# 2bitoperations/rtldavis

Measured on AMD Instinct MI355X. Metric: complex MSamples/s demodulated (uint8 IQ -> packed bits -> preamble matches -> packets), higher is better.
Workload: dtype f32 (FIR: f16 x f16 -> f32 on the matrix pipe, exact integer accumulation); 1 GPU; 4096 streams x 33 blocks x 8192 samples uint8 IQ per GPU (BASELINE configs[3]/[4]: 64 unique synthetic streams tiled, 2.21 GB resident in HBM), 14 samples/symbol, 19.2 kbit/s; streams_per_gpu=4096, parallelism=streams/1

## Files before the change

rtldavis_amd/csrc/rd_demod_mfma.hip:

```cpp
#include <cstdio>
#include <cstdlib>
#include <cstring>

#include <hip/hip_ext.h>

#include "rd_internal.h"
#include "rd_math.h"
#include "rd_mfma.h"

#define RD_MF_WG 256
#define RD_MF_WAVES (RD_MF_WG / 64)
#ifndef RD_MF_MINWAVES
#define RD_MF_MINWAVES 4
#endif
#define RD_MF_GROUP_BYTES 1152
#define RD_MF_IMG_BYTES (16 + 4 * RD_MF_GROUP_BYTES)
#define RD_MF_IMG_PAD 4624
#define RD_MF_XB_BYTES (3 * 1024 + 32 + 32)
#define RD_MF_PEND 32
#ifndef RD_MF_STAGE_TILES
#define RD_MF_STAGE_TILES 4
#endif

typedef _Float16 rd_h8 __attribute__((ext_vector_type(8)));
typedef _Float16 rd_h16 __attribute__((ext_vector_type(16)));
typedef _Float16 rd_h2 __attribute__((ext_vector_type(2)));
typedef float rd_f16v __attribute__((ext_vector_type(16)));
typedef uint32_t rd_u4v __attribute__((ext_vector_type(4)));
typedef float rd_f4v __attribute__((ext_vector_type(4)));
typedef uint32_t rd_u2v __attribute__((ext_vector_type(2)));

static const rd_mf_taps h_mf_taps = rd_mf_make_taps();
__device__ const rd_mf_taps8 g_mf_taps8 = rd_mf_make_taps8();
static const rd_mf_taps8 h_mf_taps8 = rd_mf_make_taps8();
extern "C" void rd_debug_mfma_taps8(uint16_t *out) { memcpy(out, &h_mf_taps8, sizeof h_mf_taps8); }
#ifndef RD_MF_SPARSE
#define RD_MF_SPARSE 1
#endif
constexpr bool rd_mf_taps8s_ok() { bool ok = true; (void)rd_mf_make_taps8s(&ok); return ok; }
static_assert(rd_mf_taps8s_ok(), "a row of the tap matrix has more than two non-zero elements in a group of four");
constexpr rd_mf_taps8s rd_mf_taps8s_value() { bool ok = true; return rd_mf_make_taps8s(&ok); }
__device__ const rd_mf_taps8s g_mf_taps8s = rd_mf_taps8s_value();
static const rd_mf_taps8s h_mf_taps8s = rd_mf_taps8s_value();
extern "C" void rd_debug_mfma_taps8s(uint16_t *vals, uint32_t *idx) {
    memcpy(vals, h_mf_taps8s.v, sizeof h_mf_taps8s.v);
    memcpy(idx, h_mf_taps8s.idx, sizeof h_mf_taps8s.idx);
}

extern "C" void rd_debug_mfma_taps(uint16_t *out) { memcpy(out, &h_mf_taps, sizeof h_mf_taps); }

__device__ __forceinline__ rd_h8 rd_mf_frag(rd_u2v d) {
    rd_u4v v;
    v.x = d.x & 0x00FF00FFu;
    v.y = __builtin_amdgcn_perm(0u, d.x, 0x0c030c01u);
    v.z = d.y & 0x00FF00FFu;
    v.w = __builtin_amdgcn_perm(0u, d.y, 0x0c030c01u);
    return __builtin_bit_cast(rd_h8, v);
}

__device__ __forceinline__ float rd_mf_num(float ar, float ai, float cr, float ci, float &t1) {
    t1 = ai * ci;
    return __builtin_fmaf(-ar, cr, -t1);
}
__device__ __forceinline__ float rd_mf_guard(float nmin, float tmax) { return __builtin_fmaf(-4.76837158e-7f, tmax, nmin); }


template <int OFF>
__device__ __forceinline__ void rd_lds_write16(uint32_t addr, rd_f4v v) {
    asm volatile("ds_write_b128 %0, %1 offset:%2" : : "v"(addr), "v"(v), "i"(OFF) : "memory");
}
template <int OFF>
__device__ __forceinline__ rd_f4v rd_lds_read16(uint32_t addr) {
    rd_f4v r;
    asm volatile("ds_read_b128 %0, %1 offset:%2" : "=v"(r) : "v"(addr), "i"(OFF) : "memory");
    return r;
}
__device__ __forceinline__ void rd_lds_wait(rd_f4v &r) { asm volatile("s_waitcnt lgkmcnt(0)" : "+v"(r) : : "memory"); }
__device__ __forceinline__ void rd_lds_write4(uint32_t addr, uint32_t v) {
    asm volatile("ds_write_b32 %0, %1" : : "v"(addr), "v"(v) : "memory");
}
__device__ __forceinline__ rd_u4v rd_lds_read16u(uint32_t addr) {
    rd_u4v r;
    asm volatile("ds_read_b128 %0, %1\n\ts_waitcnt lgkmcnt(0)" : "=&v"(r) : "v"(addr) : "memory");
    return r;
}
__device__ __forceinline__ uint32_t rd_lds_read4(uint32_t addr) {
    uint32_t r;
    asm volatile("ds_read_b32 %0, %1\n\ts_waitcnt lgkmcnt(0)" : "=&v"(r) : "v"(addr) : "memory");
    return r;
}
__device__ __forceinline__ uint32_t rd_lds_addr(const void *p) {
    return (uint32_t)(uintptr_t)(const __attribute__((address_space(3))) void *)p;
}

__device__ __forceinline__ bool rd_mf_any(bool c) { return __ballot(c) != 0; }


struct rd_mf8_addr {
    uint32_t xw;
    uint32_t xw7;
    uint32_t rd1, rdE, rdO;
    uint32_t rd0;
};
struct rd_mf8_kept {
    float n2, n3;
    float g0r, g0i;
    float g1r, g1i, g2r, g2i;
    float nmin, tmax;
};

template <int B>
__device__ __forceinline__ constexpr int rd_mf8_woff() { return B == 0 ? 0 : (B & 1) ? 1024 : 2048; }

template <int B, int DBG>
__device__ __forceinline__ void rd_mf8_finish(const rd_mf8_kept &k, rd_f4v &p, uint32_t &W, uint32_t &fb, bool &slow) {
    rd_lds_wait(p);
    float t0, t1;
    const float n0 = rd_mf_num(p.x, p.y, p.z, p.w, t0);
    const float n1 = rd_mf_num(p.z, p.w, k.g0r, k.g0i, t1);
    if (DBG == 0 || DBG == 3) {
        const float nm = rd_mf_guard(rd_min3abs(k.nmin, n0, n1), rd_max3abs(k.tmax, t0, t1));
        if (rd_mf_any(!(nm > RD_MF_C0_MAX))) {
            slow = true;
            float F = rd_max3abs(0.0f, p.x, p.y);
            F = rd_max3abs(F, p.z, p.w);
            F = rd_max3abs(F, k.g0r, k.g0i);
            F = rd_max3abs(F, k.g1r, k.g1i);
            F = rd_max3abs(F, k.g2r, k.g2i);
            if (!(nm > rd_mf_c0(F))) fb |= 1u << (8 * (B & 3));
        }
    }
    uint32_t w = rd_shift_in_sign(W, n0);
    w = rd_shift_in_sign(w, n1);
    w = rd_shift_in_sign(w, k.n2);
    W = __builtin_amdgcn_alignbit(w, __builtin_bit_cast(uint32_t, k.n3), 27);
}

template <int B, int DBG>
__device__ __forceinline__ void rd_mf8_block(const rd_h8 (&A)[2], const rd_f16v &dcC, const int sidx, const int sidx2, const rd_u2v (&D)[9],
                                             rd_h8 &bfA, rd_h16 &bb, const rd_mf8_addr &ad, rd_mf8_kept &k0, rd_mf8_kept &kp, rd_f4v &p, uint32_t &Wlo,
                                             uint32_t &Whi, uint32_t &fblo, uint32_t &fbhi, bool &slow, float *dg, int dleft) {
    const rd_h8 bfB = rd_mf_frag(D[B + 1]);
    if (RD_MF_SPARSE && DBG != 8 && DBG != 9) {
        const rd_h16 wB = __builtin_shufflevector(bfB, bfB, 0, 1, 2, 3, 4, 5, 6, 7, 0, 1, 2, 3, 4, 5, 6, 7);
        if (B & 1) bb = __builtin_shufflevector(wB, bb, 0, 1, 2, 3, 4, 5, 6, 7, 24, 25, 26, 27, 28, 29, 30, 31);
        else bb = __builtin_shufflevector(bb, wB, 0, 1, 2, 3, 4, 5, 6, 7, 16, 17, 18, 19, 20, 21, 22, 23);
    }
    __builtin_amdgcn_sched_barrier(0);
    rd_f16v acc;
    if (DBG == 8 || DBG == 9) {
        rd_f16v c0 = dcC;
        if (DBG == 9) asm volatile("" : "+v"(c0));
        acc = __builtin_amdgcn_mfma_f32_32x32x16_f16(A[0], bfA, c0, 0, 0, 0);
        asm volatile("" : : "v"(bfB));
    } else if (RD_MF_SPARSE) {
        const uint32_t dbits = __builtin_bit_cast(uint32_t, -(float)RD_MF_DHI / 16777216.0f);
        uint64_t dh2 = ((uint64_t)dbits << 32) | dbits;
        asm volatile("" : "+s"(dh2));
        struct { uint64_t q[8]; } ci;
#pragma unroll
        for (int i = 0; i < 4; i++) asm volatile("v_mov_b64 %0, %1" : "=v"(ci.q[i]) : "s"(dh2));
#pragma unroll
        for (int i = 4; i < 8; i++) asm volatile("v_mov_b64 %0, 0" : "=v"(ci.q[i]));
        asm volatile("s_nop 1" ::: "memory");
        const rd_f16v c0 = __builtin_bit_cast(rd_f16v, ci);
        acc = (B & 1) ? __builtin_amdgcn_smfmac_f32_32x32x32_f16(A[1], bb, c0, sidx2, 0, 0)
                      : __builtin_amdgcn_smfmac_f32_32x32x32_f16(A[0], bb, c0, sidx, 0, 0);
    } else {
        acc = __builtin_amdgcn_mfma_f32_32x32x16_f16(A[0], bfA, dcC, 0, 0, 0);
        acc = __builtin_amdgcn_mfma_f32_32x32x16_f16(A[1], bfB, acc, 0, 0, 0);
    }
    if (B >= 2) rd_mf8_finish<B - 1, DBG>(kp, p, B - 1 <= 3 ? Wlo : Whi, B - 1 <= 3 ? fblo : fbhi, slow);
    __builtin_amdgcn_sched_barrier(0);
    float g[8];
#pragma unroll
    for (int i = 0; i < 8; i++) g[i] = __builtin_fmaf(acc[i], 2048.0f, acc[8 + i]);
    if (DBG == 3) {
#pragma unroll
        for (int r = 0; r < 4; r++)
            if (8 * B + r < dleft) { dg[2 * (8 * B + r)] = g[2 * r]; dg[2 * (8 * B + r) + 1] = g[2 * r + 1]; }
    }
    if (DBG != 10 && DBG != 11) {
        const rd_f4v x = {g[4], g[5], g[6], g[7]};
        if (B == 7) rd_lds_write16<0>(ad.xw7, x);
        else rd_lds_write16<rd_mf8_woff<B>()>(ad.xw, x);
    } else {
        asm volatile("" : : "v"(g[4]), "v"(g[5]), "v"(g[6]), "v"(g[7]));
    }
    if (B >= 1 && DBG != 10 && DBG != 11) p = rd_lds_read16<0>(B == 1 ? ad.rd1 : (B & 1) ? ad.rdO : ad.rdE);
    if (DBG == 11) asm volatile("" : "+v"(p));
    rd_mf8_kept &k = B == 0 ? k0 : kp;
    float t2, t3;
    k.n2 = rd_mf_num(g[0], g[1], g[2], g[3], t2);
    k.n3 = rd_mf_num(g[2], g[3], g[4], g[5], t3);
    k.nmin = rd_min3abs(3.0e38f, k.n2, k.n3);
    k.tmax = rd_max3abs(0.0f, t2, t3);
    k.g0r = g[0]; k.g0i = g[1];
    k.g1r = g[2]; k.g1i = g[3]; k.g2r = g[4]; k.g2i = g[5];
    bfA = bfB;
}

template <int DBG>
__device__ __forceinline__ void rd_mf8_tile(const rd_h8 (&A)[2], const rd_f16v &dcC, const int sidx, const int sidx2, const rd_u2v (&D)[9],
                                            const rd_mf8_addr &ad,
                                            uint32_t &word, uint32_t &fbw, bool &slow, float *dg, int dleft) {
    rd_h8 bfA = rd_mf_frag(D[0]);
    rd_h16 bb = __builtin_shufflevector(bfA, bfA, 0, 1, 2, 3, 4, 5, 6, 7, 8, 9, 10, 11, 12, 13, 14, 15);
    rd_mf8_kept k0, kp;
    rd_f4v p = {0.0f, 0.0f, 0.0f, 0.0f};
    uint32_t Wlo = 0, Whi = 0, fblo = 0, fbhi = 0;
    slow = false;
    rd_mf8_block<0, DBG>(A, dcC, sidx, sidx2, D, bfA, bb, ad, k0, kp, p, Wlo, Whi, fblo, fbhi, slow, dg, dleft);
    rd_mf8_block<1, DBG>(A, dcC, sidx, sidx2, D, bfA, bb, ad, k0, kp, p, Wlo, Whi, fblo, fbhi, slow, dg, dleft);
    rd_mf8_block<2, DBG>(A, dcC, sidx, sidx2, D, bfA, bb, ad, k0, kp, p, Wlo, Whi, fblo, fbhi, slow, dg, dleft);
    rd_mf8_block<3, DBG>(A, dcC, sidx, sidx2, D, bfA, bb, ad, k0, kp, p, Wlo, Whi, fblo, fbhi, slow, dg, dleft);
    rd_mf8_block<4, DBG>(A, dcC, sidx, sidx2, D, bfA, bb, ad, k0, kp, p, Wlo, Whi, fblo, fbhi, slow, dg, dleft);
    rd_mf8_block<5, DBG>(A, dcC, sidx, sidx2, D, bfA, bb, ad, k0, kp, p, Wlo, Whi, fblo, fbhi, slow, dg, dleft);
    rd_mf8_block<6, DBG>(A, dcC, sidx, sidx2, D, bfA, bb, ad, k0, kp, p, Wlo, Whi, fblo, fbhi, slow, dg, dleft);
    rd_mf8_block<7, DBG>(A, dcC, sidx, sidx2, D, bfA, bb, ad, k0, kp, p, Wlo, Whi, fblo, fbhi, slow, dg, dleft);
    rd_f4v p0 = rd_lds_read16<0>(ad.rd0);
    rd_mf8_finish<7, DBG>(kp, p, Whi, fbhi, slow);
    {
        rd_lds_wait(p0);
        float t0, t1;
        const float n0 = rd_mf_num(p0.x, p0.y, p0.z, p0.w, t0);
        const float n1 = rd_mf_num(p0.z, p0.w, k0.g0r, k0.g0i, t1);
        if (DBG == 0 || DBG == 3) {
            const float nm = rd_mf_guard(rd_min3abs(k0.nmin, n0, n1), rd_max3abs(k0.tmax, t0, t1));
            if (rd_mf_any(!(nm > RD_MF_C0_MAX))) {
                slow = true;
                float F = rd_max3abs(0.0f, p0.x, p0.y);
                F = rd_max3abs(F, p0.z, p0.w);
                F = rd_max3abs(F, k0.g0r, k0.g0i);
                F = rd_max3abs(F, k0.g1r, k0.g1i);
                F = rd_max3abs(F, k0.g2r, k0.g2i);
                if (!(nm > rd_mf_c0(F))) fblo |= 1u;
            }
        }
        uint32_t b0 = rd_shift_in_sign(0u, n0);
        b0 = rd_shift_in_sign(b0, n1);
        b0 = rd_shift_in_sign(b0, k0.n2);
        b0 = __builtin_amdgcn_alignbit(b0, __builtin_bit_cast(uint32_t, k0.n3), 27);
        Wlo = (b0 << 24) | Wlo;
    }
    const uint32_t Vlo = __builtin_bitreverse32(Wlo & 0xF0F0F0F0u), Vhi = __builtin_bitreverse32(Whi & 0xF0F0F0F0u);
    const auto r = __builtin_amdgcn_permlane32_swap(Vlo, Vhi, false, false);
    word = (r[1] << 4) | r[0];
    fbw = 0;
    if (slow && rd_mf_any((fblo | fbhi) != 0)) {
        const auto f = __builtin_amdgcn_permlane32_swap(fblo, fbhi, false, false);
        fbw = f[0] | f[1];
    }
}

#ifndef RD_MF_LOAD_AUX
#define RD_MF_LOAD_AUX 2
#endif

__device__ __forceinline__ void rd_mf_issue(const rd_layout &lay, uint32_t s, uint32_t ti, uint8_t *img, int lane,
                                            bool halo_dma = true) {
    const uint8_t *src = lay.iq + (size_t)s * lay.stream_stride + (size_t)ti * RD_TILE_BYTES;
    const int perm = 8 * (lane & 7) + (lane >> 3);
    const __attribute__((address_space(1))) void *g0 = (const __attribute__((address_space(1))) void *)(src + perm * 16);
    __builtin_amdgcn_global_load_lds(g0, (__attribute__((address_space(3))) void *)(img + 16), 16, 0, RD_MF_LOAD_AUX);
    __builtin_amdgcn_global_load_lds(g0, (__attribute__((address_space(3))) void *)(img + 16 + 128), 16, 1024, RD_MF_LOAD_AUX);
    __builtin_amdgcn_global_load_lds(g0, (__attribute__((address_space(3))) void *)(img + 16 + 256), 16, 2048, RD_MF_LOAD_AUX);
    __builtin_amdgcn_global_load_lds(g0, (__attribute__((address_space(3))) void *)(img + 16 + 384), 16, 3072, RD_MF_LOAD_AUX);
    const bool has_halo = (ti > 0) || lay.hist_mode;
    if (lane == 0 && halo_dma)
        __builtin_amdgcn_global_load_lds((const __attribute__((address_space(1))) void *)(src + (has_halo ? -16 : 0)),
                                         (__attribute__((address_space(3))) void *)(img), 16, 0, 0);
}

__device__ __forceinline__ int rd_lane_now() {
    return (int)__builtin_amdgcn_mbcnt_hi(~0u, __builtin_amdgcn_mbcnt_lo(~0u, 0u));
}

__device__ __forceinline__ void rd_mf_flush(const uint32_t *pend, uint32_t count, uint32_t *fix_list, uint32_t fix_cap,
                                            uint32_t *counters, uint32_t bits_stride, uint32_t *bucket_cnt) {
    const int lane = rd_lane_now();
    asm volatile("s_waitcnt lgkmcnt(0)" ::: "memory");
    if (bucket_cnt) {
        for (uint32_t i = lane; i < count; i += 64) {
            const uint32_t e = pend[i];
            const uint32_t grp = ((e >> 4) / bits_stride) >> RD_FT_GSH;
            const uint32_t slot = atomicAdd(&bucket_cnt[grp], 1u);
            if (slot < fix_cap) fix_list[(size_t)grp * fix_cap + slot] = e;
        }
        return;
    }
    uint32_t base = 0;
    if (lane == 0) base = atomicAdd(&counters[RD_CNT_FIX], count);
    base = __builtin_amdgcn_readfirstlane(base);
    for (uint32_t i = lane; i < count; i += 64)
        if (base + i < fix_cap) fix_list[base + i] = pend[i];
}


__device__ __forceinline__ void rd_mf_store_staged(uint32_t stage_addr, uint32_t nst, uint32_t *base, uint32_t stflags) {
    const int lane = rd_lane_now();
    if (nst == RD_MF_STAGE_TILES) {
#pragma unroll
        for (int j = 0; j < RD_MF_STAGE_TILES / 4; j++) {
            const rd_u4v v = rd_lds_read16u(stage_addr + 16 * (lane + 64 * j));
            if (!(stflags & 1)) __builtin_nontemporal_store(v, (rd_u4v *)(base + 4 * (lane + 64 * j)));
            else *(rd_u4v *)(base + 4 * (lane + 64 * j)) = v;
        }
    } else {
        for (uint32_t q = 0; q < nst; q++) base[64 * q + lane] = rd_lds_read4(stage_addr + 256 * q + 4 * lane);
    }
}

struct rd_mf_pos {
    uint32_t tile, s, ti, inchunk;
};
struct rd_mf_nextchunk {
    uint32_t tile, s, ti;
};
__device__ __forceinline__ rd_mf_nextchunk rd_mf_chunk_at(uint64_t chunk_id, uint32_t chunk, uint32_t tps, uint32_t total) {
    rd_mf_nextchunk c;
    const uint32_t n_chunks = (total + chunk - 1) / chunk;
    const bool have = chunk_id < n_chunks;
    const uint32_t nt = have ? (uint32_t)chunk_id * chunk : 0u;
    c.tile = have ? nt : 0xFFFFFFFFu;
    c.s = 0; c.ti = 0;
    if (have) {
        c.s = __builtin_amdgcn_readfirstlane(c.tile / tps);
        c.ti = c.tile - c.s * tps;
    }
    return c;
}
__device__ __forceinline__ rd_mf_pos rd_mf_next(rd_mf_pos p, uint32_t chunk, uint32_t tps, const rd_mf_nextchunk &nc) {
    rd_mf_pos q;
    if (p.inchunk + 1 < chunk) {
        q.tile = p.tile + 1; q.inchunk = p.inchunk + 1;
        q.s = p.s; q.ti = p.ti + 1;
        if (q.ti >= tps) { q.ti = 0; q.s++; }
    } else {
        q.tile = nc.tile; q.inchunk = 0;
        q.s = nc.s; q.ti = nc.ti;
    }
    return q;
}

__device__ __forceinline__ void rd_mf_read_window(uint32_t a_prv, uint32_t a_own, rd_u2v (&D)[9]) {
    asm volatile("ds_read_b64 %0, %9\n\t"
                 "ds_read_b64 %1, %10\n\t"
                 "ds_read_b64 %2, %10 offset:128\n\t"
                 "ds_read_b64 %3, %10 offset:256\n\t"
                 "ds_read_b64 %4, %10 offset:384\n\t"
                 "ds_read_b64 %5, %10 offset:512\n\t"
                 "ds_read_b64 %6, %10 offset:640\n\t"
                 "ds_read_b64 %7, %10 offset:768\n\t"
                 "ds_read_b64 %8, %10 offset:896\n\t"
                 "s_waitcnt lgkmcnt(0)"
                 : "=&v"(D[0]), "=&v"(D[1]), "=&v"(D[2]), "=&v"(D[3]), "=&v"(D[4]), "=&v"(D[5]), "=&v"(D[6]),
                   "=&v"(D[7]), "=&v"(D[8])
                 : "v"(a_prv), "v"(a_own)
                 : "memory");
}

__device__ __forceinline__ uint64_t rd_stamp() {
    uint64_t t;
    __builtin_amdgcn_sched_barrier(0);
    asm volatile("s_memtime %0\n\ts_waitcnt lgkmcnt(0)" : "=s"(t) : : "memory");
    __builtin_amdgcn_sched_barrier(0);
    return t;
}
__device__ __forceinline__ uint64_t rd_stamp_real() {
    uint64_t t;
    __builtin_amdgcn_sched_barrier(0);
    asm volatile("s_memrealtime %0\n\ts_waitcnt lgkmcnt(0)" : "=s"(t) : : "memory");
    __builtin_amdgcn_sched_barrier(0);
    return t;
}


#define RD_STAMP_WORDS 12
#define RD_STF_BUCKETS 8192u
template <int DBG, bool STAMP>
__global__ __launch_bounds__(RD_MF_WG, RD_MF_MINWAVES) void k_demod_mfma(rd_layout lay, uint32_t tiles_per_stream, uint32_t total_tiles,
                                                         uint32_t chunk, uint32_t *fix_list, uint32_t fix_cap,
                                                         uint32_t *counters, float *dbg_g, uint32_t stflags) {
    __shared__ __attribute__((aligned(16))) uint8_t s_img[RD_MF_WAVES][RD_MF_IMG_PAD];
    __shared__ __attribute__((aligned(32))) uint8_t s_xb[RD_MF_WAVES][RD_MF_XB_BYTES];
    __shared__ uint32_t s_pend[RD_MF_WAVES][RD_MF_PEND];
    __shared__ __attribute__((aligned(16))) uint32_t s_stage[RD_MF_WAVES][RD_MF_STAGE_TILES][64];
    constexpr bool LOADS = DBG != 1;
    const int lane = threadIdx.x & 63;
    const int wave = __builtin_amdgcn_readfirstlane(threadIdx.x >> 6);
    uint8_t *img0 = s_img[wave];
    uint8_t *xb = s_xb[wave];
    uint32_t *mypend = s_pend[wave];
    uint32_t npend = 0;
    constexpr bool CAN_BUCKET = DBG == 0 && !STAMP;
    uint32_t *bucket_cnt = (CAN_BUCKET && (stflags & RD_STF_BUCKETS)) ? (uint32_t *)dbg_g : nullptr;

    const int n = lane & 31, h = lane >> 5;
    rd_h8 A8[2];
    rd_f16v dcC;
    int sidx = 0, sidx2 = 0;
    if (RD_MF_SPARSE && DBG != 8 && DBG != 9) {
        A8[0] = *(const rd_h8 *)g_mf_taps8s.v[lane];
        A8[1] = *(const rd_h8 *)g_mf_taps8s.v[lane ^ 32];
        sidx = (int)g_mf_taps8s.idx[lane];
        sidx2 = (int)g_mf_taps8s.idx[lane ^ 32];
    } else {
        A8[0] = *(const rd_h8 *)g_mf_taps8.v[0][lane];
        A8[1] = *(const rd_h8 *)g_mf_taps8.v[1][lane];
    }
    const float dchi = -(float)RD_MF_DHI / 16777216.0f;
#pragma unroll
    for (int i = 0; i < 16; i++) dcC[i] = i < 8 ? dchi : 0.0f;
    if (RD_MF_SPARSE && DBG != 8 && DBG != 9) asm volatile("" : "+v"(A8[0]), "+v"(A8[1]), "+v"(sidx), "+v"(sidx2));
    else asm volatile("" : "+v"(A8[0]), "+v"(A8[1]), "+v"(dcC));
    const uint32_t img_addr = rd_lds_addr(img0);
    const uint32_t own = 16 + RD_MF_GROUP_BYTES * (n >> 3) + 16 * (n & 7) + 8 * h;
    const uint32_t prv = n == 0 ? 8 * h
                       : (n & 7) ? own + 16 * 55
                                 : 16 + RD_MF_GROUP_BYTES * ((n >> 3) - 1) + 16 * 63 + 8 * h;
    const uint32_t xb_addr = rd_lds_addr(xb), pend_addr = rd_lds_addr(mypend);
    const uint32_t stage_addr = rd_lds_addr(s_stage[wave]);
    const uint32_t rtoggle = lane == 0 ? 16u : 0u, wtoggle = lane == 63 ? 16u : 0u;
    rd_mf8_addr ad8;
    ad8.xw = xb_addr + 16 * lane;
    ad8.xw7 = xb_addr + (lane == 63 ? 3072 : 1024 + 16 * lane);
    ad8.rd1 = xb_addr + (h ? 1024 + 16 * (lane - 32) : 16 * (lane + 32));
    ad8.rdE = xb_addr + (h ? 2048 + 16 * (lane - 32) : 1024 + 16 * (lane + 32));
    ad8.rdO = xb_addr + (h ? 1024 + 16 * (lane - 32) : 2048 + 16 * (lane + 32));
    ad8.rd0 = xb_addr + (h ? 16 * (lane - 32) : lane ? 1024 + 16 * (lane + 31) : 3072 + 16);
    if (lane < 8) ((uint32_t *)(xb + 3072))[lane] = 0;

    const uint32_t nwaves = gridDim.x * RD_MF_WAVES;
    const uint32_t wave_id = blockIdx.x * RD_MF_WAVES + wave;
    const bool dynamic = !(stflags & 4096) && chunk >= 4;
    uint32_t cur_chunk = wave_id;
    rd_mf_nextchunk nextc = {0xFFFFFFFFu, 0, 0};
    if (!dynamic) nextc = rd_mf_chunk_at((uint64_t)cur_chunk + nwaves, chunk, tiles_per_stream, total_tiles);
    uint32_t grab = 0;
    bool grab_pending = false;
    const uint32_t my_queue = wave_id % RD_NQUEUE;
    uint32_t *queue = &counters[RD_CNT_QUEUE0 + RD_QUEUE_STRIDE * my_queue];
    rd_mf_pos cur;
    cur.tile = wave_id * chunk;
    cur.s = cur.tile / tiles_per_stream;
    cur.ti = cur.tile % tiles_per_stream;
    cur.inchunk = 0;
    rd_mf_pos nx1 = rd_mf_next(cur, chunk, tiles_per_stream, nextc);

    uint32_t nst = 0;
    uint32_t *st_base = nullptr;
    bool st_flush = false;
    uint64_t sm_wait = 0, sm_gap = 0, sm_comp = 0, sm_wait_st = 0, sm_t0 = 0, sm_r0 = 0, sm_mark = 0, sm_wmax = 0;
    uint32_t sm_iters = 0, sm_iters_st = 0;
    bool sm_stored = false;
    if (STAMP) { sm_t0 = rd_stamp(); sm_r0 = rd_stamp_real(); }
    if (LOADS && cur.tile < total_tiles) rd_mf_issue(lay, cur.s, cur.ti, img0, lane);
    if (STAMP) sm_mark = rd_stamp();
    while (cur.tile < total_tiles) {
        const uint32_t tile = cur.tile, s = cur.s, ti = cur.ti, inchunk = cur.inchunk;
        uint64_t sm_a = 0;
        if (STAMP) { sm_a = rd_stamp(); sm_comp += sm_a - sm_mark; }
        asm volatile("s_waitcnt vmcnt(0)" : "+v"(grab) : : "memory");
        uint64_t sm_b = 0;
        if (STAMP) {
            sm_b = rd_stamp();
            const uint64_t w = sm_b - sm_a;
            sm_wait += w;
            if (w > sm_wmax) sm_wmax = w;
            if (sm_stored) { sm_wait_st += w; sm_iters_st++; }
            sm_iters++;
            sm_stored = false;
        }
        if (dynamic) {
            if (grab_pending) {
                nextc = rd_mf_chunk_at((uint64_t)nwaves + my_queue + (uint64_t)RD_NQUEUE * __builtin_amdgcn_readfirstlane(grab),
                                       chunk, tiles_per_stream, total_tiles);
                grab_pending = false;
            }
            if (inchunk == 0) {
                const uint32_t one = 1, zoff = 0;
                uint64_t saved_exec;
                asm volatile("s_mov_b64 %1, exec\n\ts_mov_b64 exec, 1\n\tglobal_atomic_add %0, %2, %3, %4 sc0\n\ts_mov_b64 exec, %1"
                             : "+v"(grab), "=&s"(saved_exec) : "v"(zoff), "v"(one), "s"(queue) : "memory");
                grab_pending = true;
            }
        } else if (inchunk == 0 && tile != wave_id * chunk) {
            cur_chunk += nwaves;
            nextc = rd_mf_chunk_at((uint64_t)cur_chunk + nwaves, chunk, tiles_per_stream, total_tiles);
        }
        if (!(stflags & 4)) __builtin_amdgcn_s_setprio(3);
        rd_u2v D[9];
        rd_mf_read_window(img_addr + prv, img_addr + own, D);
        if (nst == RD_MF_STAGE_TILES || (nst && st_flush)) {
            rd_mf_store_staged(stage_addr, nst, st_base, stflags);
            nst = 0;
            if (STAMP) sm_stored = true;
        }
        const rd_mf_pos nx2 = rd_mf_next(nx1, chunk, tiles_per_stream, nextc);
        bool halo_dma = true;
        {
            const bool follows = nx1.tile < total_tiles && nx1.s == s && nx1.ti == ti + 1;
            if (follows) {
                halo_dma = false;
                if (n == 31) asm volatile("ds_write_b64 %0, %1" : : "v"(img_addr + 8 * h), "v"(D[8]) : "memory");
            }
        }
        if (LOADS && nx1.tile < total_tiles) rd_mf_issue(lay, nx1.s, nx1.ti, img0, lane, halo_dma);
        if (!(stflags & 4)) __builtin_amdgcn_s_setprio(0);
        if (STAMP) { sm_mark = rd_stamp(); sm_gap += sm_mark - sm_b; }

        uint32_t word = 0;
        bool slow_taken = false;
        uint32_t fbw8 = 0;
        if (DBG == 2 || DBG == 6) {
#pragma unroll
            for (int j = 0; j < 9; j++) word ^= D[j].x ^ D[j].y;
        } else {
            float *dg = DBG == 3 ? dbg_g + ((size_t)tile * RD_TILE_SAMPLES + 64 * n + 4 * h + 1) * 2 : nullptr;
            const int dleft = RD_TILE_SAMPLES - (64 * n + 4 * h + 1);
            rd_mf8_tile<DBG>(A8, dcC, sidx, sidx2, D, ad8, word, fbw8, slow_taken, dg, dleft);
            ad8.rd0 ^= rtoggle;
            ad8.xw7 ^= wtoggle;
        }
        uint32_t gmask = 0;
        const bool carry = inchunk > 0 && ti > 0;
        const uint32_t run = ti * 64 + 2 * n + h;
        const uint32_t t0 = run * RD_RUN;
        const bool any_flag = slow_taken && rd_mf_any(fbw8 != 0);
        if (any_flag) gmask = ((fbw8 * 0x00204081u) >> 21) & 0xFu;
        if (!carry && lane == 0) {
            if (ti == 0 && !lay.hist_mode) gmask = 0xFu;
            else gmask |= 1u;
        }
        const bool ragged = (ti + 1 == tiles_per_stream) && (lay.n_samples % RD_TILE_SAMPLES) != 0;
        if (DBG == 6) {
            if (word == 0x12345678u) lay.bits[0] = word;
        } else if (!ragged) {
            if (nst == 0) {
                st_base = &lay.bits[(size_t)s * lay.bits_stride + ti * 64];
                if (stflags & 2) st_base = &lay.bits[(((size_t)s * lay.bits_stride + ti * 64) & 0x3FFFFu) & ~255u];
            }
            rd_lds_write4(stage_addr + 256 * nst + 4 * (2 * n + h), word);
            nst++;
            const bool next_ragged = (nx1.ti + 1 == tiles_per_stream) && (lay.n_samples % RD_TILE_SAMPLES) != 0;
            st_flush = !(nx1.tile < total_tiles && nx1.s == s && nx1.ti == ti + 1 && !next_ragged);
        } else if (t0 < lay.n_samples) {
            const uint32_t left = lay.n_samples - t0;
            if (left < RD_RUN) {
                word &= (1u << left) - 1u;
                gmask &= (1u << ((left + RD_GROUP - 1) / RD_GROUP)) - 1u;
            }
            lay.bits[(size_t)s * lay.bits_stride + run] = word;
        } else {
            gmask = 0;
        }
        if (DBG == 1 || DBG == 2 || DBG == 6) gmask = 0;
        const uint64_t fm = (any_flag || !carry) ? __ballot(gmask != 0) : 0;
        if (fm) {
            const uint32_t nf = (uint32_t)__popcll(fm);
            if (npend + nf > RD_MF_PEND) {
                rd_mf_flush(mypend, npend, fix_list, fix_cap, counters, (uint32_t)lay.bits_stride, bucket_cnt);
                npend = 0;
            }
            if (gmask)
                rd_lds_write4(pend_addr + 4 * (npend + __builtin_amdgcn_mbcnt_hi((uint32_t)(fm >> 32),
                                                                                  __builtin_amdgcn_mbcnt_lo((uint32_t)fm, 0))),
                              ((uint32_t)((size_t)s * lay.bits_stride + run) << 4) | gmask);
            npend += nf;
        }
        cur = nx1;
        nx1 = nx2;
    }
    if (nst) rd_mf_store_staged(stage_addr, nst, st_base, stflags);
    if (npend) rd_mf_flush(mypend, npend, fix_list, fix_cap, counters, (uint32_t)lay.bits_stride, bucket_cnt);
    if (STAMP && dbg_g) {
        const uint64_t t1 = rd_stamp(), r1 = rd_stamp_real();
        sm_comp += t1 - sm_mark;
        if (lane == 0) {
            uint64_t *o = (uint64_t *)dbg_g + (size_t)wave_id * RD_STAMP_WORDS;
            o[0] = sm_wait; o[1] = sm_gap; o[2] = sm_comp; o[3] = sm_wait_st;
            o[4] = sm_iters; o[5] = sm_iters_st; o[6] = t1 - sm_t0; o[7] = r1 - sm_r0;
            o[8] = sm_wmax; o[9] = sm_r0; o[10] = r1;
            uint32_t xcc;
            asm volatile("s_getreg_b32 %0, hwreg(HW_REG_XCC_ID)" : "=s"(xcc));
            o[11] = xcc;
        }
    }
}

static int rd_mf_env(const char *name, int dflt) {
    const char *e = getenv(name);
    return e ? atoi(e) : dflt;
}

struct rd_mf_params {
    int dbg = 0, stamp = 0, chunk_env = 0, per_cu_env = 0, n_cu = 256;
    uint32_t stflags = 0;
    rd_mf_params() {
        chunk_env = rd_mf_env("RD_K1_CHUNK", 0);
        per_cu_env = rd_mf_env("RD_K1_WGS_PER_CU", 0);
#ifdef RD_DIAG
        dbg = rd_mf_env("RD_K1_DEBUG", 0);
        stamp = rd_mf_env("RD_K1_STAMPS", 0) ? 1 : 0;
        stflags = (uint32_t)rd_mf_env("RD_K1_STFLAGS", 0) & (1u | 2u | 4u | 4096u);
#endif
        int dev = 0;
        hipDeviceProp_t prop;
        if (hipGetDevice(&dev) == hipSuccess && hipGetDeviceProperties(&prop, dev) == hipSuccess && prop.multiProcessorCount > 0)
            n_cu = prop.multiProcessorCount;
    }
};
static const rd_mf_params &rd_mf_get_params() {
    static const rd_mf_params p;
    return p;
}

#ifdef RD_DIAG
static uint64_t *g_stamp_buf = nullptr;
static uint32_t g_stamp_waves = 0;
extern "C" int rd_diag_read_stamps(uint64_t *out, uint32_t cap_waves, uint32_t *n_waves) {
    if (!g_stamp_buf || !n_waves) return RD_ERR_STATE;
    if (hipDeviceSynchronize() != hipSuccess) return RD_ERR_DEVICE;
    *n_waves = g_stamp_waves;
    const uint32_t n = g_stamp_waves < cap_waves ? g_stamp_waves : cap_waves;
    if (n && hipMemcpy(out, g_stamp_buf, (size_t)n * RD_STAMP_WORDS * 8, hipMemcpyDeviceToHost) != hipSuccess) return RD_ERR_DEVICE;
    return RD_OK;
}
extern "C" int rd_diag_variant(int *dbg, int *stamp, uint32_t *stflags) {
    const rd_mf_params &P = rd_mf_get_params();
    if (dbg) *dbg = P.dbg;
    if (stamp) *stamp = P.stamp;
    if (stflags) *stflags = P.stflags;
    return RD_OK;
}
#endif

struct rd_mf_launch_args {
    rd_layout lay;
    uint32_t tps, total;
    uint64_t total64;
// ... 145 lines not shown
```

rtldavis_amd/csrc/rd_kernels.hip:

```cpp
#include <algorithm>
#include <cstdlib>

#include <hip/hip_ext.h>

#include "rd_internal.h"
#include "rd_math.h"
#include "rd_mfma.h"
#include "rd_parse.h"

uint32_t rd_launch_demod(const rd_layout &lay, uint32_t *fix_list, uint32_t fix_cap, uint32_t *counters, hipStream_t st,
                         hipEvent_t ev_start, hipEvent_t ev_stop, uint32_t flags, uint32_t *chunk_out, uint32_t *bucket_cnt) {
    if (!bucket_cnt) flags &= ~RD_DEMOD_FIX_BUCKETS;
    const bool bucketed = rd_launch_demod_mfma(lay, fix_list, fix_cap, counters, st, ev_start, ev_stop, nullptr, flags, chunk_out, bucket_cnt);
    return bucketed ? RD_DEMOD_FIX_BUCKETS : 0u;
}

__global__ __launch_bounds__(256) void k_fixup(rd_layout lay, uint32_t runs_per_stream, const uint32_t *fix_list,
                                               uint32_t fix_cap, const uint32_t *counters, int all,
                                               uint32_t *zero_next, uint32_t zero_words) {
    if (zero_next && blockIdx.x == 0)
        for (uint32_t i = threadIdx.x; i < zero_words; i += blockDim.x) zero_next[i] = 0;
    uint64_t count;
    if (all) {
        count = (uint64_t)lay.n_streams * runs_per_stream;
// ... 791 lines not shown
}

#define RD_FT_WG 256
#ifndef RD_FT_DEPTH
#define RD_FT_DEPTH 5
#endif
struct rd_ft_args {
    rd_layout lay;
    rd_devcfg cfg;
    int n_calls;
    int p_hi;
    int skip_fix;
    const uint32_t *fixb;
    const uint32_t *fixcnt;
    uint32_t fix_bcap;
    uint32_t bcap;
    uint32_t bucket_limit;
    uint32_t *gstate;
    uint32_t seq;
    rd_packet *recs;
    uint32_t rec_cap;
    uint32_t *counters;
    uint32_t *zero_next;
    uint32_t zero_words;
    uint64_t *stamps;
    int abl;
};
#ifdef RD_DIAG
#define RD_FT_STAMP(k) do { if (a.stamps && (tid & 63) == 0) { uint64_t t_; asm volatile("s_memrealtime %0\n\ts_waitcnt lgkmcnt(0)" : "=s"(t_) : : "memory"); \
                                                               a.stamps[(size_t)grp * 8 + (k)] = t_; } } while (0)
#else
#define RD_FT_STAMP(k) do { } while (0)
#endif

template <int S_, int T>
__device__ __forceinline__ uint32_t rd_tap(const uint32_t *r, int o) {
    constexpr int wj = (T * S_) >> 5, sh = (T * S_) & 31;
    return sh ? __builtin_amdgcn_alignbit(r[o + wj + 1], r[o + wj], sh) : r[o + wj];
}
constexpr int rd_tt3(bool pa, bool pb, bool pc) { return (pa ? 0xF0 : 0x0F) & (pb ? 0xCC : 0x33) & (pc ? 0xAA : 0x55); }
template <int S_, int P_, uint64_t PRE_, int T>
__device__ __forceinline__ uint32_t rd_match_from(uint32_t m, const uint32_t *r, int o) {
    if constexpr (T >= P_) {
        return m;
    } else if constexpr (T + 1 == P_) {
        const uint32_t v = rd_tap<S_, T>(r, o);
        return __builtin_amdgcn_bitop3_b32(m, v, v, rd_tt3(true, (PRE_ >> T) & 1, (PRE_ >> T) & 1));
    } else {
        const uint32_t n = __builtin_amdgcn_bitop3_b32(m, rd_tap<S_, T>(r, o), rd_tap<S_, T + 1>(r, o),
                                                       rd_tt3(true, (PRE_ >> T) & 1, (PRE_ >> (T + 1)) & 1));
        return rd_match_from<S_, P_, PRE_, T + 2>(n, r, o);
    }
}
template <int S_, int P_, uint64_t PRE_>
__device__ __forceinline__ uint32_t rd_match_word(const uint32_t *r, int o) {
    static_assert(P_ >= 3, "three taps in the first instruction");
    const uint32_t m = __builtin_amdgcn_bitop3_b32(rd_tap<S_, 0>(r, o), rd_tap<S_, 1>(r, o), rd_tap<S_, 2>(r, o),
                                                   rd_tt3(PRE_ & 1, (PRE_ >> 1) & 1, (PRE_ >> 2) & 1));
    return rd_match_from<S_, P_, PRE_, 3>(m, r, o);
}

__device__ __forceinline__ void rd_barrier_lds() { asm volatile("s_waitcnt lgkmcnt(0)\n\ts_barrier" ::: "memory"); }

template <int S_, int P_, uint64_t PRE_, int K_>
__global__ __launch_bounds__(RD_FT_WG, 4) void k_tail(rd_ft_args a) {
    constexpr int G = RD_FT_STREAMS;
    static_assert(PRE_ & 1, "positions below 0 are skipped because the preamble starts with a one");
    static_assert(RD_FT_WG == 64 * G, "one wave per stream in the classify strips");
    extern __shared__ __attribute__((aligned(16))) uint32_t s_dyn[];
    uint32_t *s_t = s_dyn;
    int32_t *s_pos = (int32_t *)(s_dyn + (size_t)G * a.bcap * 8);
    uint32_t *s_ord = s_dyn + (size_t)G * a.bcap * 9;
    __shared__ uint32_t s_cnt[G], s_kept[G];
    __shared__ uint32_t s_ready;
    const int tid = threadIdx.x, lane = tid & 63, wave = __builtin_amdgcn_readfirstlane(tid >> 6);
    const int grp = blockIdx.x, n_groups = gridDim.x;
    const int stream0 = grp * G;
    const int n_here = a.lay.n_streams - stream0 < G ? a.lay.n_streams - stream0 : G;
    const int nwords = (int)((a.lay.n_samples + 31) / 32);
    if (grp == 0 && a.zero_next)
        for (uint32_t i = tid; i < a.zero_words; i += RD_FT_WG) a.zero_next[i] = 0;
    if (tid < G) { s_cnt[tid] = 0; s_kept[tid] = 0; }
    if (tid == 0) s_ready = 0;
    const int prio_q = (int)(((unsigned)grp * 4u) / (unsigned)n_groups);
    if (wave == 0) RD_FT_STAMP(0);

    uint32_t n_fix_raw = 0;
    if (!a.skip_fix) {
        const uint32_t *bk = a.fixb + (size_t)grp * a.fix_bcap;
        const uint32_t e_first = (uint32_t)tid < a.fix_bcap ? bk[tid] : 0u;
        n_fix_raw = a.fixcnt[grp];
        const uint32_t n_fix = n_fix_raw < a.fix_bcap ? n_fix_raw : a.fix_bcap;
        uint32_t *s_items = s_t;
        __shared__ uint32_t s_nitems;
        static_assert(RD_GROUPS == 4, "an entry lists up to four groups");
        for (uint32_t i0 = 0; i0 < n_fix; i0 += RD_FT_WG) {
            if (tid == 0) s_nitems = 0;
            __syncthreads();
            const uint32_t i = i0 + (uint32_t)tid;
            const uint32_t e = i < n_fix ? (i0 == 0 ? e_first : bk[i]) : 0u;
            const uint32_t k = (uint32_t)__popc(e & 0xFu);
            if (k) {
                uint32_t at = atomicAdd(&s_nitems, k);
                for (int g = 0; g < RD_GROUPS; g++)
                    if ((e >> g) & 1) s_items[at++] = ((uint32_t)tid << 2) | (uint32_t)g;
                s_items[4 * RD_FT_WG + tid] = e;
            }
            __syncthreads();
            const uint32_t n_items = s_nitems;
            for (uint32_t it = (uint32_t)tid; it < n_items; it += RD_FT_WG) {
                const uint32_t item = s_items[it];
                const uint32_t ee = s_items[4 * RD_FT_WG + (item >> 2)];
                const int g = (int)(item & 3u);
                const uint32_t widx = ee >> 4;
                const uint32_t s = widx / (uint32_t)a.lay.bits_stride;
                const uint32_t run = widx - s * (uint32_t)a.lay.bits_stride;
                const uint8_t *base = a.lay.iq + (size_t)s * a.lay.stream_stride;
                const long t0 = (long)run * RD_RUN + g * RD_GROUP;
                const long left = (long)a.lay.n_samples - t0;
                if (left <= 0) continue;
                const int count = left < RD_GROUP ? (int)left : RD_GROUP;
                const uint8_t *p = base + 2 * (t0 - 10);
                uint32_t dw[10];
                const long x = a.lay.valid_from - (t0 - 10), z = (long)a.lay.n_samples + 8 - (t0 - 10);
                const int d_lo = x <= 0 ? 0 : x >= 20 ? 10 : (int)(x / 2);
                const int d_hi = z <= 0 ? 0 : z >= 20 ? 10 : (int)((z + 1) / 2);
#pragma unroll
                for (int d = 0; d < 10; d++) dw[d] = (d >= d_lo && d < d_hi) ? *(const uint32_t *)(p + 4 * d) : 0u;
                ((uint8_t *)a.lay.bits)[(size_t)widx * 4 + g] = (uint8_t)rd_exact_group_dw(dw, t0, count, a.lay.valid_from);
            }
            if (i0 + RD_FT_WG < n_fix) __syncthreads();
        }
    }
    __syncthreads();
    if (wave == 0) RD_FT_STAMP(1);

    {
        constexpr int NW = ((RD_SEARCH_OUT + ((P_ - 1) * S_ + 31) / 32 + 1 + 3) / 4) * 4;
        const int gps = a.p_hi / (32 * RD_SEARCH_OUT) + 1;
        const int wgps = (gps + 63) / 64;
        const int units = n_here * wgps;
        auto fetch = [&](int g, int rem, uint32_t (&r)[NW]) {
            const int gi = rem * 64 + lane;
            const uint32_t *w = a.lay.bits + (size_t)(stream0 + g) * a.lay.bits_stride;
            int w0 = RD_SEARCH_OUT * gi;
            w0 = w0 + NW <= nwords ? w0 : nwords - NW;
#pragma unroll
            for (int j = 0; j < NW / 4; j++) {
                const uint4 v4 = *(const uint4 *)(w + w0 + 4 * j);
                r[4 * j] = v4.x; r[4 * j + 1] = v4.y; r[4 * j + 2] = v4.z; r[4 * j + 3] = v4.w;
            }
        };
        auto test = [&](int g, int rem, const uint32_t (&r)[NW]) {
            const int gi = rem * 64 + lane;
            uint32_t m[RD_SEARCH_OUT] = {};
            const int p0 = 32 * RD_SEARCH_OUT * gi;
            if (gi < gps) {
#pragma unroll
                for (int o = 0; o < RD_SEARCH_OUT; o++) m[o] = rd_match_word<S_, P_, PRE_>(r, o);
                if (p0 + 32 * RD_SEARCH_OUT - 1 > a.p_hi) {
#pragma unroll
                    for (int o = 0; o < RD_SEARCH_OUT; o++) {
                        const int q0 = p0 + 32 * o;
                        if (q0 + 31 > a.p_hi) m[o] &= (a.p_hi < q0) ? 0u : (0xFFFFFFFFu >> (31 - (a.p_hi - q0)));
                    }
                }
            }
            uint32_t anym = 0;
#pragma unroll
            for (int o = 0; o < RD_SEARCH_OUT; o++) anym |= m[o];
            if (__ballot(anym != 0)) {
                uint32_t mine = 0;
#pragma unroll
                for (int o = 0; o < RD_SEARCH_OUT; o++) mine += (uint32_t)__popc(m[o]);
                uint32_t incl = mine;
#pragma unroll
                for (int sh = 1; sh < 64; sh <<= 1) {
                    const uint32_t up = (uint32_t)__shfl_up((int)incl, sh, 64);
                    if (lane >= sh) incl += up;
                }
                const uint32_t tot = (uint32_t)__shfl((int)incl, 63, 64);
                uint32_t slot0 = 0;
                if (lane == 0) slot0 = atomicAdd(&s_cnt[g], tot);
                uint32_t slot = (uint32_t)__builtin_amdgcn_readfirstlane((int)slot0) + incl - mine;
#pragma unroll
                for (int o = 0; o < RD_SEARCH_OUT; o++) {
                    uint32_t mm = m[o];
                    while (mm) {
                        const int bpos = __builtin_ctz(mm);
                        mm &= mm - 1;
                        if (slot < a.bcap) s_pos[(size_t)g * a.bcap + slot] = p0 + 32 * o + bpos;
                        slot++;
                    }
                }
            }
        };
        constexpr int DEPTH = RD_FT_DEPTH;
        uint32_t rb[DEPTH][NW];
        const int dq = G / wgps, dr = G % wgps;
        int fg = wave / wgps, fr = wave % wgps, fu = wave;
        int tg = fg, tr = fr, prio_k = 0;
        auto step = [&](int &gg, int &rr) { gg += dq; rr += dr; if (rr >= wgps) { rr -= wgps; gg++; } };
        auto fetch_next = [&](uint32_t (&r)[NW]) {
#ifdef RD_DIAG
            if (a.abl & 2) return;
#endif
            fetch(fg, fr, r);
            if (fu + G < units) { fu += G; step(fg, fr); }
        };
        auto test_next = [&](const uint32_t (&r)[NW]) {
#ifdef RD_DIAG
            if (a.abl & 1) { if (r[0] == 0x12345678u) s_cnt[0] = 1; step(tg, tr); return; }
#endif
            switch ((prio_q + prio_k++) & 3) {
                case 0: __builtin_amdgcn_s_setprio(0); break;
                case 1: __builtin_amdgcn_s_setprio(1); break;
                case 2: __builtin_amdgcn_s_setprio(2); break;
// ... 1140 lines not shown
```

Measured before the change: 2.005 million MS/s.

## Precompute tile-boundary carry via extra MFMA instead of forcing exact fix for chunk starts

When a wave starts a new chunk at a non-zero tile, it now DMAs two 16-byte halo blocks before the tile and runs a small MFMA prologue to rebuild the filter carry state. That state is written into the crossing buffer, so the first group no longer has to be forced onto the slow exact-fix list. The halo-forwarding condition is tightened to the same chunk. In the follow-up kernel, a full barrier is skipped when there are no fix entries, and the fix count is read as wave-uniform. The cost is an extra MFMA pass and LDS traffic per chunk start, in exchange for fewer fix entries and less serialized exact recomputation.

```diff
diff --git a/rtldavis_amd/csrc/rd_demod_mfma.hip b/rtldavis_amd/csrc/rd_demod_mfma.hip
--- a/rtldavis_amd/csrc/rd_demod_mfma.hip
+++ b/rtldavis_amd/csrc/rd_demod_mfma.hip
@@ -15,7 +15,8 @@
 #endif
 #define RD_MF_GROUP_BYTES 1152
 #define RD_MF_IMG_BYTES (16 + 4 * RD_MF_GROUP_BYTES)
-#define RD_MF_IMG_PAD 4624
+#define RD_MF_IMG_FRONT 16
+#define RD_MF_IMG_PAD (RD_MF_IMG_FRONT + 4624)
 #define RD_MF_XB_BYTES (3 * 1024 + 32 + 32)
 #define RD_MF_PEND 32
 #ifndef RD_MF_STAGE_TILES
@@ -91,6 +92,10 @@
 }
 __device__ __forceinline__ uint32_t rd_lds_addr(const void *p) {
     return (uint32_t)(uintptr_t)(const __attribute__((address_space(3))) void *)p;
+}
+
+__device__ __forceinline__ int rd_lane_now() {
+    return (int)__builtin_amdgcn_mbcnt_hi(~0u, __builtin_amdgcn_mbcnt_lo(~0u, 0u));
 }
 
 __device__ __forceinline__ bool rd_mf_any(bool c) { return __ballot(c) != 0; }
@@ -253,9 +258,36 @@
     }
 }
 
+template <int DBG>
+__device__ __forceinline__ void rd_mf8_pre(const rd_h8 (&A)[2], const rd_f16v &dcC, const int sidx, const rd_u2v (&E)[2],
+                                           uint32_t carry_addr) {
+    const rd_h8 f0 = rd_mf_frag(E[0]), f1 = rd_mf_frag(E[1]);
+    rd_f16v acc;
+    if (RD_MF_SPARSE) {
+        const rd_h16 bb = __builtin_shufflevector(f0, f1, 0, 1, 2, 3, 4, 5, 6, 7, 8, 9, 10, 11, 12, 13, 14, 15);
+        const float dchi = -(float)RD_MF_DHI / 16777216.0f;
+        rd_f16v c0;
+#pragma unroll
+        for (int i = 0; i < 16; i++) c0[i] = i < 8 ? dchi : 0.0f;
+        acc = __builtin_amdgcn_smfmac_f32_32x32x32_f16(A[0], bb, c0, sidx, 0, 0);
+    } else {
+        acc = __builtin_amdgcn_mfma_f32_32x32x16_f16(A[0], f0, dcC, 0, 0, 0);
+        acc = __builtin_amdgcn_mfma_f32_32x32x16_f16(A[1], f1, acc, 0, 0, 0);
+    }
+    rd_f4v x;
+#pragma unroll
+    for (int i = 0; i < 4; i++) x[i] = __builtin_fmaf(acc[4 + i], 2048.0f, acc[12 + i]);
+    if (rd_lane_now() == 63) {
+        rd_lds_write16<0>(carry_addr, x);
+        rd_lds_write16<16>(carry_addr, x);
+    }
+}
+
 #ifndef RD_MF_LOAD_AUX
 #define RD_MF_LOAD_AUX 2
 #endif
+
+__device__ __forceinline__ bool rd_mf_has_pre(uint32_t ti) { return ti > 0; }
 
 __device__ __forceinline__ void rd_mf_issue(const rd_layout &lay, uint32_t s, uint32_t ti, uint8_t *img, int lane,
                                             bool halo_dma = true) {
@@ -267,13 +299,10 @@
     __builtin_amdgcn_global_load_lds(g0, (__attribute__((address_space(3))) void *)(img + 16 + 256), 16, 2048, RD_MF_LOAD_AUX);
     __builtin_amdgcn_global_load_lds(g0, (__attribute__((address_space(3))) void *)(img + 16 + 384), 16, 3072, RD_MF_LOAD_AUX);
     const bool has_halo = (ti > 0) || lay.hist_mode;
-    if (lane == 0 && halo_dma)
-        __builtin_amdgcn_global_load_lds((const __attribute__((address_space(1))) void *)(src + (has_halo ? -16 : 0)),
-                                         (__attribute__((address_space(3))) void *)(img), 16, 0, 0);
-}
-
-__device__ __forceinline__ int rd_lane_now() {
-    return (int)__builtin_amdgcn_mbcnt_hi(~0u, __builtin_amdgcn_mbcnt_lo(~0u, 0u));
+    const int back = rd_mf_has_pre(ti) ? 16 * (2 - lane) : has_halo ? 16 : 0;
+    if (lane < 2 && halo_dma)
+        __builtin_amdgcn_global_load_lds((const __attribute__((address_space(1))) void *)(src - back),
+                                         (__attribute__((address_space(3))) void *)(img - RD_MF_IMG_FRONT), 16, 0, 0);
 }
 
 __device__ __forceinline__ void rd_mf_flush(const uint32_t *pend, uint32_t count, uint32_t *fix_list, uint32_t fix_cap,
@@ -389,7 +418,7 @@
     constexpr bool LOADS = DBG != 1;
     const int lane = threadIdx.x & 63;
     const int wave = __builtin_amdgcn_readfirstlane(threadIdx.x >> 6);
-    uint8_t *img0 = s_img[wave];
+    uint8_t *img0 = s_img[wave] + RD_MF_IMG_FRONT;
     uint8_t *xb = s_xb[wave];
     uint32_t *mypend = s_pend[wave];
     uint32_t npend = 0;
@@ -448,6 +477,7 @@
     cur.inchunk = 0;
     rd_mf_pos nx1 = rd_mf_next(cur, chunk, tiles_per_stream, nextc);
 
+    constexpr bool PRE = DBG == 0 || DBG == 3 || DBG == 7;
     uint32_t nst = 0;
     uint32_t *st_base = nullptr;
     bool st_flush = false;
@@ -490,6 +520,12 @@
             nextc = rd_mf_chunk_at((uint64_t)cur_chunk + nwaves, chunk, tiles_per_stream, total_tiles);
         }
         if (!(stflags & 4)) __builtin_amdgcn_s_setprio(3);
+        if (PRE && !(inchunk > 0 && ti > 0) && rd_mf_has_pre(ti)) {
+            rd_u2v E[2];
+            asm volatile("ds_read_b64 %0, %2\n\tds_read_b64 %1, %2 offset:16\n\ts_waitcnt lgkmcnt(0)"
+                         : "=&v"(E[0]), "=&v"(E[1]) : "v"(img_addr - RD_MF_IMG_FRONT + 8 * (rd_lane_now() >> 5)) : "memory");
+            rd_mf8_pre<DBG>(A8, dcC, sidx, E, xb_addr + 3072);
+        }
         rd_u2v D[9];
         rd_mf_read_window(img_addr + prv, img_addr + own, D);
         if (nst == RD_MF_STAGE_TILES || (nst && st_flush)) {
@@ -499,12 +535,10 @@
         }
         const rd_mf_pos nx2 = rd_mf_next(nx1, chunk, tiles_per_stream, nextc);
         bool halo_dma = true;
-        {
-            const bool follows = nx1.tile < total_tiles && nx1.s == s && nx1.ti == ti + 1;
-            if (follows) {
-                halo_dma = false;
-                if (n == 31) asm volatile("ds_write_b64 %0, %1" : : "v"(img_addr + 8 * h), "v"(D[8]) : "memory");
-            }
+        const bool follows = nx1.inchunk > 0 && nx1.tile < total_tiles && nx1.s == s && nx1.ti == ti + 1;
+        if (follows) {
+            halo_dma = false;
+            if (n == 31) asm volatile("ds_write_b64 %0, %1" : : "v"(img_addr + 8 * h), "v"(D[8]) : "memory");
         }
         if (LOADS && nx1.tile < total_tiles) rd_mf_issue(lay, nx1.s, nx1.ti, img0, lane, halo_dma);
         if (!(stflags & 4)) __builtin_amdgcn_s_setprio(0);
@@ -525,11 +559,12 @@
         }
         uint32_t gmask = 0;
         const bool carry = inchunk > 0 && ti > 0;
+        const bool forced = !carry && !(PRE && rd_mf_has_pre(ti));
         const uint32_t run = ti * 64 + 2 * n + h;
         const uint32_t t0 = run * RD_RUN;
         const bool any_flag = slow_taken && rd_mf_any(fbw8 != 0);
         if (any_flag) gmask = ((fbw8 * 0x00204081u) >> 21) & 0xFu;
-        if (!carry && lane == 0) {
+        if (forced && lane == 0) {
             if (ti == 0 && !lay.hist_mode) gmask = 0xFu;
             else gmask |= 1u;
         }
@@ -556,7 +591,7 @@
             gmask = 0;
         }
         if (DBG == 1 || DBG == 2 || DBG == 6) gmask = 0;
-        const uint64_t fm = (any_flag || !carry) ? __ballot(gmask != 0) : 0;
+        const uint64_t fm = (any_flag || forced) ? __ballot(gmask != 0) : 0;
         if (fm) {
             const uint32_t nf = (uint32_t)__popcll(fm);
             if (npend + nf > RD_MF_PEND) {
diff --git a/rtldavis_amd/csrc/rd_kernels.hip b/rtldavis_amd/csrc/rd_kernels.hip
--- a/rtldavis_amd/csrc/rd_kernels.hip
+++ b/rtldavis_amd/csrc/rd_kernels.hip
@@ -897,15 +897,18 @@
         for (uint32_t i = tid; i < a.zero_words; i += RD_FT_WG) a.zero_next[i] = 0;
     if (tid < G) { s_cnt[tid] = 0; s_kept[tid] = 0; }
     if (tid == 0) s_ready = 0;
+    rd_barrier_lds();
     const int prio_q = (int)(((unsigned)grp * 4u) / (unsigned)n_groups);
     if (wave == 0) RD_FT_STAMP(0);
 
     uint32_t n_fix_raw = 0;
+    bool fixed_any = false;
     if (!a.skip_fix) {
         const uint32_t *bk = a.fixb + (size_t)grp * a.fix_bcap;
         const uint32_t e_first = (uint32_t)tid < a.fix_bcap ? bk[tid] : 0u;
-        n_fix_raw = a.fixcnt[grp];
+        n_fix_raw = (uint32_t)__builtin_amdgcn_readfirstlane((int)a.fixcnt[grp]);
         const uint32_t n_fix = n_fix_raw < a.fix_bcap ? n_fix_raw : a.fix_bcap;
+        fixed_any = n_fix != 0;
         uint32_t *s_items = s_t;
         __shared__ uint32_t s_nitems;
         static_assert(RD_GROUPS == 4, "an entry lists up to four groups");
@@ -947,7 +950,7 @@
             if (i0 + RD_FT_WG < n_fix) __syncthreads();
         }
     }
-    __syncthreads();
+    if (fixed_any) __syncthreads();
     if (wave == 0) RD_FT_STAMP(1);
 
     {
```

Result: no change. 2.002 million MS/s (-0.2%).
